# boundless-xyz/boundless

Hardware: AMD Instinct MI355X
Metric: segment-proofs/sec @ 2^20 cycles (higher is better)
Workload: dtype u32 (BabyBear Montgomery)

## Files before the change

boundless_amd/csrc/circuit_dev.hpp:

```cpp
#pragma once
#include <type_traits>

#include "circuit.hpp"
#include "fp.hpp"
#include "poseidon2_arith.hpp"

namespace bx {
inline namespace BX_MAD_FLAVOUR {

constexpr i64 FINAL_MAX = ((i64)(P / 2) - 1) * ((i64)1 << 32);
static_assert(ub(FINAL_MAX) < (i64)P && FINAL_MAX <= SREDC_MAX, "FINAL_MAX");

template <int V>
struct IntC {
    static constexpr int value = V;
};
template <int BEGIN, int END, class F>
BX_HD void static_for(F&& f) {
    if constexpr (BEGIN < END) {
        f(IntC<BEGIN>{});
        static_for<BEGIN + 1, END>(f);
    }
}

template <int TT, int GG>
struct ConsPlan {
    static constexpr int NPOOL = (int)Circuit::POOL;
    static constexpr i64 BC = (i64)(P / 2);
    static constexpr i64 chain_bound() {
        i64 y = BC;
        for (int f = 2; f + 1 < GG; ++f) y = ub(y * BC);
        return y;
    }
    static constexpr i64 TERM = chain_bound() * BC;
    static constexpr int ISZ = (int)(SREDC_MAX / TERM) < 4 ? (int)(SREDC_MAX / TERM) : 4;
    static_assert(ISZ >= 1 && ISZ * TERM <= SREDC_MAX, "cons_sum: inner group beyond sredc's range");

    int nq = 0, no = 0, n2 = 0;
    int first[TT]{}, len[TT]{}, term[TT][ISZ]{};
    int obeg[TT + 1]{}, lbeg[TT + 1]{};
    i64 max_inner = 0, max_outer = 0, max_l2 = 0, max_l3 = 0;

    constexpr ConsPlan() {
        for (int g = 0; g < TT; ++g)
            for (int a = 0; a < NPOOL; ++a) {
                int members[TT]{}, n = 0;
                for (int t = 0; t < TT; ++t)
                    if ((int)Circuit::pool_idx((unsigned)t, 0u) == a) members[n++] = t;
                const int groups = (n + ISZ - 1) / ISZ;
                if (g >= groups) continue;
                const int sz = n / groups + (g < n % groups ? 1 : 0), at = g * (n / groups) + (g < n % groups ? g : n % groups);
                first[nq] = a;
                len[nq] = sz;
                for (int k = 0; k < sz; ++k) term[nq][k] = members[at + k];
                if (sz * TERM > max_inner) max_inner = sz * TERM;
                ++nq;
            }
        i64 rb[TT + 1]{};
        i64 cur = 0;
        for (int q = 0; q < nq; ++q) {
            const i64 add = ub(len[q] * TERM) * BC;
            if (q > 0 && cur + add > SREDC_MAX) {
                rb[no++] = ub(cur);
                obeg[no] = q;
                cur = 0;
            }
            cur += add;
            if (cur > max_outer) max_outer = cur;
        }
        rb[no++] = ub(cur);
        obeg[no] = nq;
        cur = 0;
        for (int o = 0; o < no; ++o) {
            const i64 add = rb[o] * (i64)MONT_ONE;
            if (o > 0 && cur + add > FINAL_MAX) {
                max_l3 += ub(cur) * (i64)MONT_ONE;
                lbeg[++n2] = o;
                cur = 0;
            }
            cur += add;
            if (cur > max_l2) max_l2 = cur;
        }
        max_l3 += ub(cur) * (i64)MONT_ONE;
        lbeg[++n2] = no;
    }
};
template <int TT, int GG>
inline constexpr ConsPlan<TT, GG> cons_plan{};

template <int TT>
struct PairPlan {
    static constexpr int NPOOL = (int)Circuit::POOL, NID = NPOOL * NPOOL;
    static constexpr i64 BC = (i64)(P / 2);
    static constexpr i64 PAIR = ub(BC * BC);
    static constexpr i64 TERM = PAIR * PAIR;
    static constexpr int GRP = (int)(SREDC_MAX / TERM);
    static_assert(GRP == 3 && GRP * TERM <= SREDC_MAX, "cons_sum: pair group beyond sredc's range");
    static constexpr int pair_id(unsigned a, unsigned b) { return a < b ? (int)(a * NPOOL + b) : (int)(b * NPOOL + a); }

    int np = 0, ng = 0, n2 = 0;
    int pa[2 * TT]{}, pb[2 * TT]{};
    int seq[TT]{}, s1[TT]{}, s2[TT]{};
    int pbeg[TT + 1]{};
    int gbeg[TT + 1]{}, lbeg[TT + 1]{};
    int max_live = 0;
    i64 max_group = 0, max_l2 = 0, max_l3 = 0;

    constexpr PairPlan() {
        int sp[TT][3][2]{}, pop[NID]{}, ref[NID]{}, ch[TT]{};
        for (int t = 0; t < TT; ++t) {
            unsigned x[4]{};
            for (unsigned f = 0; f < 4; ++f) x[f] = Circuit::pool_idx((unsigned)t, f);
            for (int s = 0; s < 3; ++s) {
                sp[t][s][0] = pair_id(x[0], x[s + 1]);
                sp[t][s][1] = pair_id(x[s == 0 ? 2 : 1], x[s == 2 ? 2 : 3]);
                ++pop[sp[t][s][0]];
                ++pop[sp[t][s][1]];
            }
        }
        for (int t = 0; t < TT; ++t) {
            for (int s = 1; s < 3; ++s)
                if (pop[sp[t][s][0]] + pop[sp[t][s][1]] > pop[sp[t][ch[t]][0]] + pop[sp[t][ch[t]][1]]) ch[t] = s;
            ++ref[sp[t][ch[t]][0]];
            ++ref[sp[t][ch[t]][1]];
        }
        for (int sweep = 0; sweep < 4; ++sweep)
            for (int t = 0; t < TT; ++t) {
                --ref[sp[t][ch[t]][0]];
                --ref[sp[t][ch[t]][1]];
                int best = 0, best_new = 3, best_ref = 0;
                for (int s = 0; s < 3; ++s) {
                    const int a = sp[t][s][0], b = sp[t][s][1];
                    const int fresh = (ref[a] == 0) + (ref[b] == 0 && b != a), shared = ref[a] + ref[b];
                    if (fresh < best_new || (fresh == best_new && shared > best_ref)) best = s, best_new = fresh, best_ref = shared;
                }
                ch[t] = best;
                ++ref[sp[t][best][0]];
                ++ref[sp[t][best][1]];
            }
        for (int pass = 0; pass < 2; ++pass) {
            int snap[NID]{};
            for (int i = 0; i < NID; ++i) snap[i] = ref[i];
            for (int r = 1; r <= 4; ++r)
                for (int p = 0; p < NID; ++p) {
                    if (snap[p] != r || ref[p] == 0 || ref[p] > 4) continue;
                    int users[4]{}, was[4]{}, nu = 0, moved = 0, delta = 0;
                    for (int t = 0; t < TT; ++t)
                        if (sp[t][ch[t]][0] == p || sp[t][ch[t]][1] == p) users[nu++] = t;
                    for (int u = 0; u < nu; ++u) {
                        was[u] = ch[users[u]];
                        for (int k = 0; k < 2; ++k) delta -= (--ref[sp[users[u]][was[u]][k]] == 0);
                    }
                    for (; moved < nu; ++moved) {
                        const int t = users[moved];
                        int best = -1, best_new = 3, best_ref = 0;
                        for (int s = 0; s < 3; ++s) {
                            const int a = sp[t][s][0], b = sp[t][s][1];
                            if (a == p || b == p) continue;
                            const int fresh = (ref[a] == 0) + (ref[b] == 0 && b != a), shared = ref[a] + ref[b];
                            if (best < 0 || fresh < best_new || (fresh == best_new && shared > best_ref)) best = s, best_new = fresh, best_ref = shared;
                        }
                        if (best < 0) break;
                        ch[t] = best;
                        for (int k = 0; k < 2; ++k) delta += (ref[sp[t][best][k]]++ == 0);
                    }
                    if (moved < nu || delta > 0 || (delta == 0 && pass == 0)) {
                        for (int u = 0; u < moved; ++u)
                            for (int k = 0; k < 2; ++k) --ref[sp[users[u]][ch[users[u]]][k]];
                        for (int u = 0; u < nu; ++u) {
                            ch[users[u]] = was[u];
                            for (int k = 0; k < 2; ++k) ++ref[sp[users[u]][was[u]][k]];
                        }
                    }
                }
        }
        int num[NID]{}, live = 0, glen = 0, gp[2 * GRP]{};
        bool placed[TT]{};
        for (int i = 0; i < NID; ++i) num[i] = -1;
        for (int slot = 0; slot < TT;) {
            int best = -1, best_new = 3, best_last = -1;
            if (glen < GRP)
                for (int t = 0; t < TT; ++t) {
                    if (placed[t]) continue;
                    const int a = sp[t][ch[t]][0], b = sp[t][ch[t]][1];
                    bool clash = false;
                    for (int k = 0; k < 2 * glen; ++k) clash = clash || gp[k] == a || gp[k] == b;
                    if (clash) continue;
                    const int fresh = (num[a] < 0) + (num[b] < 0 && b != a);
                    const int last = a == b ? (ref[a] == 2) : (ref[a] == 1) + (ref[b] == 1);
                    if (fresh < best_new || (fresh == best_new && last > best_last)) best = t, best_new = fresh, best_last = last;
                }
            if (best < 0) {
                gbeg[++ng] = slot;
                glen = 0;
                continue;
            }
            const int a = sp[best][ch[best]][0], b = sp[best][ch[best]][1];
            for (int k = 0; k < 2; ++k) {
                const int id = k ? b : a;
                if (num[id] < 0) {
                    num[id] = np;
                    pa[np] = id / NPOOL;
                    pb[np] = id % NPOOL;
                    ++np;
                    ++live;
                }
            }
            if (live > max_live) max_live = live;
            live -= (--ref[a] == 0);
            live -= (--ref[b] == 0);
            placed[best] = true;
            seq[slot] = best;
            s1[slot] = num[a];
            s2[slot] = num[b];
            gp[2 * glen] = a;
            gp[2 * glen + 1] = b;
            ++glen;
            pbeg[++slot] = np;
        }
        gbeg[++ng] = TT;
        i64 cur = 0;
        for (int g = 0; g < ng; ++g) {
            const i64 sum = (gbeg[g + 1] - gbeg[g]) * TERM, add = ub(sum) * (i64)MONT_ONE;
            if (sum > max_group) max_group = sum;
            if (g > 0 && cur + add > FINAL_MAX) {
                max_l3 += ub(cur) * (i64)MONT_ONE;
                lbeg[++n2] = g;
                cur = 0;
            }
            cur += add;
            if (cur > max_l2) max_l2 = cur;
        }
        max_l3 += ub(cur) * (i64)MONT_ONE;
        lbeg[++n2] = ng;
    }
};
template <int TT>
inline constexpr PairPlan<TT> pair_plan{};

BX_HD i64 smad_r(i32 r, i64 c, int alt = 0) {
#if defined(__HIP_DEVICE_COMPILE__) && defined(BX_PLAIN_MAD)
    (void)alt;
    i32 k = (i32)MONT_ONE;
    asm volatile("" : "+s"(k));
    return (i64)r * (i64)k + c;
#else
    return smad_k(r, MONT_ONE, c, alt);
#endif
}

template <int TT, int GG>
BX_HD uint32_t cons_sum(const i32 (&pool)[Circuit::POOL], uint32_t , uint32_t ) {
    static_assert(TT > 0 && GG > 0, "cons_sum: the run-time form takes a canonical pool");
#pragma unroll
    for (unsigned i = 0; i < Circuit::POOL; ++i) BX_ASSERT_BOUND(pool[i] <= (i32)(P / 2) && pool[i] >= -(i32)(P / 2), "cons_sum: a pool entry that is not centred");
    if constexpr (GG == 4) {
        constexpr int N2 = pair_plan<TT>.n2;
        static_assert(pair_plan<TT>.max_group <= SREDC_MAX, "cons_sum: a group sum beyond sredc's range");
        static_assert(pair_plan<TT>.max_l2 <= FINAL_MAX && pair_plan<TT>.max_l3 <= FINAL_MAX, "cons_sum: term count beyond the three reduction levels");
        i32 pr[pair_plan<TT>.np];
        i64 acc3 = 0;
        i32 result = 0;
        static_for<0, N2>([&](auto lc) {
            constexpr int l = decltype(lc)::value;
            i64 acc2 = 0;
            static_for<pair_plan<TT>.lbeg[l], pair_plan<TT>.lbeg[l + 1]>([&](auto gc) {
                constexpr int g = decltype(gc)::value;
                i64 acc = 0;
                static_for<pair_plan<TT>.gbeg[g], pair_plan<TT>.gbeg[g + 1]>([&](auto sc) {
                    constexpr int s = decltype(sc)::value;
                    static_for<pair_plan<TT>.pbeg[s], pair_plan<TT>.pbeg[s + 1]>([&](auto pc) {
                        constexpr int p = decltype(pc)::value;
                        pr[p] = sredc(smul(pool[pair_plan<TT>.pa[p]], pool[pair_plan<TT>.pb[p]], p), p);
                        BX_ASSERT_BOUND(pr[p] <= PairPlan<TT>::PAIR && pr[p] >= -PairPlan<TT>::PAIR, "cons_sum pair");
                    });
                    acc = smad(pr[pair_plan<TT>.s1[s]], pr[pair_plan<TT>.s2[s]], acc, s);
                });
                acc2 = smad_r(sredc(acc, 3), acc2, g);
            });
            BX_ASSERT_BOUND(acc2 <= FINAL_MAX && acc2 >= -FINAL_MAX, "cons_sum second level");
            const i32 r2 = sredc(acc2, 2);
            if constexpr (N2 == 1) result = r2;
            else acc3 = smad_r(r2, acc3, l);
        });
        if constexpr (N2 > 1) {
            BX_ASSERT_BOUND(acc3 <= FINAL_MAX && acc3 >= -FINAL_MAX, "cons_sum third level");
            result = sredc(acc3, 0);
        }
        return (uint32_t)(result + (result < 0 ? (i32)P : 0));
    } else if constexpr (GG >= 3) {
        constexpr int N2 = cons_plan<TT, GG>.n2;
        static_assert(cons_plan<TT, GG>.max_inner <= SREDC_MAX && cons_plan<TT, GG>.max_outer <= SREDC_MAX, "cons_sum: a group sum beyond sredc's range");
        static_assert(cons_plan<TT, GG>.max_l2 <= FINAL_MAX && cons_plan<TT, GG>.max_l3 <= FINAL_MAX, "cons_sum: term count beyond the three reduction levels");
        i64 acc3 = 0;
        i32 result = 0;
        static_for<0, N2>([&](auto lc) {
            constexpr int l = decltype(lc)::value;
            i64 acc2 = 0;
            static_for<cons_plan<TT, GG>.lbeg[l], cons_plan<TT, GG>.lbeg[l + 1]>([&](auto oc) {
                constexpr int o = decltype(oc)::value;
                i64 outer = 0;
                static_for<cons_plan<TT, GG>.obeg[o], cons_plan<TT, GG>.obeg[o + 1]>([&](auto qc) {
                    constexpr int q = decltype(qc)::value;
                    i64 inner = 0;
                    static_for<0, cons_plan<TT, GG>.len[q]>([&](auto kc) {
                        constexpr int k = decltype(kc)::value;
                        constexpr unsigned t = (unsigned)cons_plan<TT, GG>.term[q][k];
                        i32 y = pool[Circuit::pool_idx(t, 1u)];
#pragma unroll
                        for (int f = 2; f + 1 < GG; ++f) y = sredc(smul(y, pool[Circuit::pool_idx(t, (unsigned)f)], f), f);
                        inner = smad(y, pool[Circuit::pool_idx(t, (unsigned)(GG - 1))], inner, k);
                    });
                    outer = smad(sredc(inner, 3), pool[cons_plan<TT, GG>.first[q]], outer, q);
                });
                acc2 = smad_r(sredc(outer, 1), acc2, o);
            });
            const i32 r2 = sredc(acc2, 2);
            if constexpr (N2 == 1) result = r2;
            else acc3 = smad_r(r2, acc3, l);
        });
        if constexpr (N2 > 1) result = sredc(acc3, 0);
        return (uint32_t)(result + (result < 0 ? (i32)P : 0));
    } else {
        static_assert(TT <= 3 * 8 * 7 && GG >= 1, "cons_sum: term count beyond the three reduction levels");
        constexpr int GRP = 3, NG = (TT + GRP - 1) / GRP;
        i64 acc2 = 0, acc3 = 0;
        i32 result = 0;
#pragma unroll
        for (int g = 0; g < NG; ++g) {
            const int nk = (g + 1) * GRP <= TT ? GRP : TT - g * GRP;
            i64 acc = 0;
#pragma unroll
            for (int k = 0; k < GRP; ++k) {
                if (k < nk) {
                    const i32 x = pool[Circuit::pool_idx((unsigned)(g * GRP + k), 0u)];
                    if constexpr (GG == 1) acc = smad_k(x, MONT_ONE, acc, k);
                    else acc = smad(x, pool[Circuit::pool_idx((unsigned)(g * GRP + k), 1u)], acc, k);
                }
            }
            const i32 r = sredc(acc, 3);
            acc2 = smad_r(r, acc2, g);
            if ((g & 7) == 7 || g == NG - 1) {
                const i32 r2 = sredc(acc2, 1);
                acc2 = 0;
                if constexpr (NG <= 8) result = r2;
                else acc3 = smad_r(r2, acc3, 2);
            }
        }
        if constexpr (NG > 8) result = sredc(acc3, 0);
        return (uint32_t)(result + (result < 0 ? (i32)P : 0));
    }
}

template <int TT, int GG>
BX_HD uint32_t cons_sum(const uint32_t (&pool_u)[Circuit::POOL], uint32_t T, uint32_t G) {
    if constexpr (TT > 0) {
        i32 pool[Circuit::POOL];
#pragma unroll
        for (unsigned i = 0; i < Circuit::POOL; ++i) pool[i] = fp_centre(pool_u[i]);
        return cons_sum<TT, GG>(pool, T, G);
    } else {
        uint32_t sum = 0;
        for (uint32_t t = 0; t < T; ++t) {
            uint32_t prod = pool_u[Circuit::pool_idx(t, 0u)];
            for (uint32_t f = 1; f < G; ++f) prod = fp_mul(prod, pool_u[Circuit::pool_idx(t, f)]);
            sum = fp_add(sum, prod);
        }
        return sum;
    }
}

template <bool CENTRED>
struct DerivedRegs {
    using word = std::conditional_t<CENTRED, i32, uint32_t>;
    BX_HD static word enter(uint32_t v) {
        if constexpr (CENTRED) return fp_centre(v);
        else return v;
    }
    word ring[8], u[3], k[4];
    BX_HD void fill(word (&pool)[Circuit::POOL], word slot1) const {
        pool[0] = u[0]; pool[1] = slot1; pool[2] = u[1]; pool[3] = u[2];
#pragma unroll
        for (int q = 0; q < 8; ++q) pool[4 + q] = ring[q];
#pragma unroll
        for (int q = 0; q < 4; ++q) pool[12 + q] = k[q];
    }
    BX_HD void shift(word d, word next_u, word next_k) {
#pragma unroll
        for (int q = 7; q > 0; --q) ring[q] = ring[q - 1];
        ring[0] = d;
        u[0] = u[1]; u[1] = u[2]; u[2] = next_u;
        k[0] = k[1]; k[1] = k[2]; k[2] = k[3]; k[3] = next_k;
    }
};

}
}
```

Baseline: 30.41.

## Replace multi-level sredc reduction trees in cons_sum with folded i64 accumulator chains

Rewrites all three cons_sum branches (GG==4, GG>=3, GG<=2) to keep one long i64 accumulator chain. Overflow is controlled by a cheap fold_r step, which multiplies the high 32 bits by MONT_ONE and adds the low word, instead of a full sredc at each level. New constexpr planners (FoldPlan, cut_segments) schedule pair products into segments and prove the bounds statically. This removes most intermediate Montgomery reductions in constraint evaluation, but it makes one serial dependence chain where independent group accumulators used to exist, which may lower instruction-level parallelism.

```diff
diff --git a/boundless_amd/csrc/circuit_dev.hpp b/boundless_amd/csrc/circuit_dev.hpp
--- a/boundless_amd/csrc/circuit_dev.hpp
+++ b/boundless_amd/csrc/circuit_dev.hpp
@@ -40,6 +40,8 @@
     int first[TT]{}, len[TT]{}, term[TT][ISZ]{};
     int obeg[TT + 1]{}, lbeg[TT + 1]{};
     i64 max_inner = 0, max_outer = 0, max_l2 = 0, max_l3 = 0;
+    int nf = 0, fbeg[TT + 1]{};
+    i64 max_fchain = 0, max_ftotal = 0;
 
     constexpr ConsPlan() {
         for (int g = 0; g < TT; ++g)
@@ -83,6 +85,27 @@
         }
         max_l3 += ub(cur) * (i64)MONT_ONE;
         lbeg[++n2] = no;
+        const int fewest = cut_segments(nq);
+        if (cut_segments((nq + fewest - 1) / fewest) > fewest) cut_segments(nq);
+    }
+    constexpr int cut_segments(int cap) {
+        i64 cur = 0;
+        nf = 0;
+        max_fchain = 0;
+        for (int q = 0; q < nq; ++q) {
+            const i64 add = ub(len[q] * TERM) * BC;
+            bool again = false;
+            for (int r = fbeg[nf]; r < q; ++r) again = again || first[r] == first[q];
+            if (q > 0 && (again || q - fbeg[nf] >= cap || cur > INT64_MAX - add)) {
+                fbeg[++nf] = q;
+                cur = fold_ub(cur);
+            }
+            cur += add;
+            if (cur > max_fchain) max_fchain = cur;
+        }
+        fbeg[++nf] = nq;
+        max_ftotal = fold_ub(cur);
+        return nf;
     }
 };
 template <int TT, int GG>
@@ -238,6 +261,93 @@
 template <int TT>
 inline constexpr PairPlan<TT> pair_plan{};
 
+template <int TT, int NCH_ = 1>
+struct FoldPlan {
+    static constexpr int SEG = 5, NCH = NCH_;
+    static constexpr i64 TERM = PairPlan<TT>::TERM;
+    static constexpr i64 STEADY = (SEG * TERM + (i64)MONT_ONE + ((i64)1 << 32)) / 15 * 16 + 16;
+    static_assert(NCH >= 1 && STEADY < INT64_MAX && fold_ub(STEADY) + SEG * TERM <= STEADY, "cons_sum: the chain bound is not invariant below 2^63");
+
+    int np = 0, ns = 0;
+    int pa[2 * TT]{}, pb[2 * TT]{};
+    int seq[TT]{}, s1[TT]{}, s2[TT]{};
+    int pbeg[TT + 1]{};
+    int sbeg[TT + 1]{};
+    int max_live = 0;
+    i64 max_chain = 0, max_total = 0;
+
+    constexpr FoldPlan() {
+        const PairPlan<TT>& pp = pair_plan<TT>;
+        int ta[TT]{}, tb[TT]{}, ref[2 * TT]{}, num[2 * TT]{};
+        for (int s = 0; s < TT; ++s) {
+            ta[pp.seq[s]] = pp.s1[s];
+            tb[pp.seq[s]] = pp.s2[s];
+            ++ref[pp.s1[s]];
+            ++ref[pp.s2[s]];
+        }
+        for (int i = 0; i < 2 * TT; ++i) num[i] = -1;
+        int live = 0, glen = 0, gp[2 * SEG]{};
+        bool placed[TT]{};
+        for (int slot = 0; slot < TT;) {
+            int best = -1, best_new = 3, best_last = -1, best_due = 0;
+            const int segs_left = (TT - slot + glen + SEG - 1) / SEG;
+            if (glen < SEG)
+                for (int t = 0; t < TT; ++t) {
+                    if (placed[t]) continue;
+                    const int a = ta[t], b = tb[t];
+                    bool clash = false;
+                    for (int k = 0; k < 2 * glen; ++k) clash = clash || gp[k] == a || gp[k] == b;
+                    if (clash) continue;
+                    const int most = ref[a] > ref[b] ? ref[a] : ref[b], due = most >= segs_left ? most : 0;
+                    const int fresh = (num[a] < 0) + (num[b] < 0 && b != a);
+                    const int last = a == b ? (ref[a] == 2) : (ref[a] == 1) + (ref[b] == 1);
+                    if (due > best_due || (due == best_due && (fresh < best_new || (fresh == best_new && last > best_last))))
+                        best = t, best_new = fresh, best_last = last, best_due = due;
+                }
+            if (best < 0) {
+                sbeg[++ns] = slot;
+                glen = 0;
+                continue;
+            }
+            const int a = ta[best], b = tb[best];
+            for (int k = 0; k < 2; ++k) {
+                const int id = k ? b : a;
+                if (num[id] < 0) {
+                    num[id] = np;
+                    pa[np] = pp.pa[id];
+                    pb[np] = pp.pb[id];
+                    ++np;
+                    ++live;
+                }
+            }
+            if (live > max_live) max_live = live;
+            live -= (--ref[a] == 0);
+            live -= (--ref[b] == 0);
+            placed[best] = true;
+            seq[slot] = best;
+            s1[slot] = num[a];
+            s2[slot] = num[b];
+            gp[2 * glen] = a;
+            gp[2 * glen + 1] = b;
+            ++glen;
+            pbeg[++slot] = np;
+        }
+        sbeg[++ns] = TT;
+        i64 chain[NCH]{};
+        for (int g = 0; g < ns; ++g) {
+            i64& a = chain[g % NCH];
+            a = (g < NCH ? 0 : fold_ub(a)) + (sbeg[g + 1] - sbeg[g]) * TERM;
+            if (a > max_chain) max_chain = a;
+        }
+        for (int c = 0; c < NCH && c < ns; ++c) max_total += fold_ub(chain[c]);
+    }
+};
+template <int TT, int NCH = 1>
+inline constexpr FoldPlan<TT, NCH> fold_plan{};
+constexpr int FOLD_CHAINS = 1;
+template <int TT>
+inline constexpr FoldPlan<TT, FOLD_CHAINS> cons_fold{};
+
 BX_HD i64 smad_r(i32 r, i64 c, int alt = 0) {
 #if defined(__HIP_DEVICE_COMPILE__) && defined(BX_PLAIN_MAD)
     (void)alt;
@@ -249,105 +359,97 @@
 #endif
 }
 
+BX_HD i64 fold_r(i64 a, int alt = 0) {
+    BX_ASSERT_BOUND(a >= -INT64_MAX, "fold_r operand");
+    const i64 r = smad_r((i32)(a >> 32), (i64)(uint32_t)a, alt);
+    BX_ASSERT_BOUND(iabs64(r) <= iabs64(a) / 16 + ((i64)1 << 32) + (i64)MONT_ONE, "fold_r result");
+    return r;
+}
+BX_HD i64 smad_chain(i32 a, i32 b, i64 c, int alt = 0) {
+#if defined(__HIP_DEVICE_COMPILE__) && defined(BX_PLAIN_MAD)
+    (void)alt;
+    i64 r = (i64)a * (i64)b + c;
+    asm("" : "+v"(r));
+    return r;
+#else
+    return smad(a, b, c, alt);
+#endif
+}
+
 template <int TT, int GG>
 BX_HD uint32_t cons_sum(const i32 (&pool)[Circuit::POOL], uint32_t , uint32_t ) {
     static_assert(TT > 0 && GG > 0, "cons_sum: the run-time form takes a canonical pool");
 #pragma unroll
     for (unsigned i = 0; i < Circuit::POOL; ++i) BX_ASSERT_BOUND(pool[i] <= (i32)(P / 2) && pool[i] >= -(i32)(P / 2), "cons_sum: a pool entry that is not centred");
     if constexpr (GG == 4) {
-        constexpr int N2 = pair_plan<TT>.n2;
-        static_assert(pair_plan<TT>.max_group <= SREDC_MAX, "cons_sum: a group sum beyond sredc's range");
-        static_assert(pair_plan<TT>.max_l2 <= FINAL_MAX && pair_plan<TT>.max_l3 <= FINAL_MAX, "cons_sum: term count beyond the three reduction levels");
-        i32 pr[pair_plan<TT>.np];
-        i64 acc3 = 0;
-        i32 result = 0;
-        static_for<0, N2>([&](auto lc) {
-            constexpr int l = decltype(lc)::value;
-            i64 acc2 = 0;
-            static_for<pair_plan<TT>.lbeg[l], pair_plan<TT>.lbeg[l + 1]>([&](auto gc) {
-                constexpr int g = decltype(gc)::value;
-                i64 acc = 0;
-                static_for<pair_plan<TT>.gbeg[g], pair_plan<TT>.gbeg[g + 1]>([&](auto sc) {
-                    constexpr int s = decltype(sc)::value;
-                    static_for<pair_plan<TT>.pbeg[s], pair_plan<TT>.pbeg[s + 1]>([&](auto pc) {
-                        constexpr int p = decltype(pc)::value;
-                        pr[p] = sredc(smul(pool[pair_plan<TT>.pa[p]], pool[pair_plan<TT>.pb[p]], p), p);
-                        BX_ASSERT_BOUND(pr[p] <= PairPlan<TT>::PAIR && pr[p] >= -PairPlan<TT>::PAIR, "cons_sum pair");
-                    });
-                    acc = smad(pr[pair_plan<TT>.s1[s]], pr[pair_plan<TT>.s2[s]], acc, s);
+        using Plan = FoldPlan<TT, FOLD_CHAINS>;
+        constexpr int NCH = Plan::NCH < cons_fold<TT>.ns ? Plan::NCH : cons_fold<TT>.ns;
+        static_assert(cons_fold<TT>.max_chain <= Plan::STEADY, "cons_sum: a chain beyond its steady-state bound");
+        static_assert(cons_fold<TT>.max_total <= FINAL_MAX, "cons_sum: the folded chains beyond the last reduction's range");
+        i32 pr[cons_fold<TT>.np];
+        i64 chain[NCH];
+        static_for<0, cons_fold<TT>.ns>([&](auto gc) {
+            constexpr int g = decltype(gc)::value, c = g % Plan::NCH;
+            static_for<cons_fold<TT>.sbeg[g], cons_fold<TT>.sbeg[g + 1]>([&](auto sc) {
+                constexpr int s = decltype(sc)::value;
+                static_for<cons_fold<TT>.pbeg[s], cons_fold<TT>.pbeg[s + 1]>([&](auto pc) {
+                    constexpr int p = decltype(pc)::value;
+                    pr[p] = sredc(smul(pool[cons_fold<TT>.pa[p]], pool[cons_fold<TT>.pb[p]], p), p);
+                    BX_ASSERT_BOUND(pr[p] <= PairPlan<TT>::PAIR && pr[p] >= -PairPlan<TT>::PAIR, "cons_sum pair");
                 });
-                acc2 = smad_r(sredc(acc, 3), acc2, g);
+                if constexpr (s > cons_fold<TT>.sbeg[g]) chain[c] = smad_chain(pr[cons_fold<TT>.s1[s]], pr[cons_fold<TT>.s2[s]], chain[c], s);
+                else if constexpr (g >= Plan::NCH) chain[c] = smad_chain(pr[cons_fold<TT>.s1[s]], pr[cons_fold<TT>.s2[s]], fold_r(chain[c], g), s);
+                else chain[c] = smul(pr[cons_fold<TT>.s1[s]], pr[cons_fold<TT>.s2[s]], s);
             });
-            BX_ASSERT_BOUND(acc2 <= FINAL_MAX && acc2 >= -FINAL_MAX, "cons_sum second level");
-            const i32 r2 = sredc(acc2, 2);
-            if constexpr (N2 == 1) result = r2;
-            else acc3 = smad_r(r2, acc3, l);
+            BX_ASSERT_BOUND(chain[c] <= cons_fold<TT>.max_chain && chain[c] >= -cons_fold<TT>.max_chain, "cons_sum chain");
         });
-        if constexpr (N2 > 1) {
-            BX_ASSERT_BOUND(acc3 <= FINAL_MAX && acc3 >= -FINAL_MAX, "cons_sum third level");
-            result = sredc(acc3, 0);
-        }
+        i64 total = fold_r(chain[0], 0);
+        static_for<1, NCH>([&](auto cc) { total += fold_r(chain[decltype(cc)::value], decltype(cc)::value); });
+        BX_ASSERT_BOUND(total <= cons_fold<TT>.max_total && total >= -cons_fold<TT>.max_total, "cons_sum folded chains");
+        const i32 result = sredc(total, 0);
         return (uint32_t)(result + (result < 0 ? (i32)P : 0));
     } else if constexpr (GG >= 3) {
-        constexpr int N2 = cons_plan<TT, GG>.n2;
-        static_assert(cons_plan<TT, GG>.max_inner <= SREDC_MAX && cons_plan<TT, GG>.max_outer <= SREDC_MAX, "cons_sum: a group sum beyond sredc's range");
-        static_assert(cons_plan<TT, GG>.max_l2 <= FINAL_MAX && cons_plan<TT, GG>.max_l3 <= FINAL_MAX, "cons_sum: term count beyond the three reduction levels");
-        i64 acc3 = 0;
-        i32 result = 0;
-        static_for<0, N2>([&](auto lc) {
-            constexpr int l = decltype(lc)::value;
-            i64 acc2 = 0;
-            static_for<cons_plan<TT, GG>.lbeg[l], cons_plan<TT, GG>.lbeg[l + 1]>([&](auto oc) {
-                constexpr int o = decltype(oc)::value;
-                i64 outer = 0;
-                static_for<cons_plan<TT, GG>.obeg[o], cons_plan<TT, GG>.obeg[o + 1]>([&](auto qc) {
-                    constexpr int q = decltype(qc)::value;
-                    i64 inner = 0;
-                    static_for<0, cons_plan<TT, GG>.len[q]>([&](auto kc) {
-                        constexpr int k = decltype(kc)::value;
-                        constexpr unsigned t = (unsigned)cons_plan<TT, GG>.term[q][k];
-                        i32 y = pool[Circuit::pool_idx(t, 1u)];
+        static_assert(cons_plan<TT, GG>.max_inner <= SREDC_MAX, "cons_sum: a group sum beyond sredc's range");
+        static_assert(cons_plan<TT, GG>.max_ftotal <= FINAL_MAX, "cons_sum: the folded chain beyond the last reduction's range");
+        i64 chain = 0;
+        static_for<0, cons_plan<TT, GG>.nf>([&](auto fc) {
+            constexpr int f = decltype(fc)::value;
+            static_for<cons_plan<TT, GG>.fbeg[f], cons_plan<TT, GG>.fbeg[f + 1]>([&](auto qc) {
+                constexpr int q = decltype(qc)::value;
+                i64 inner = 0;
+                static_for<0, cons_plan<TT, GG>.len[q]>([&](auto kc) {
+                    constexpr int k = decltype(kc)::value;
+                    constexpr unsigned t = (unsigned)cons_plan<TT, GG>.term[q][k];
+                    i32 y = pool[Circuit::pool_idx(t, 1u)];
 #pragma unroll
-                        for (int f = 2; f + 1 < GG; ++f) y = sredc(smul(y, pool[Circuit::pool_idx(t, (unsigned)f)], f), f);
-                        inner = smad(y, pool[Circuit::pool_idx(t, (unsigned)(GG - 1))], inner, k);
-                    });
-                    outer = smad(sredc(inner, 3), pool[cons_plan<TT, GG>.first[q]], outer, q);
+                    for (int g = 2; g + 1 < GG; ++g) y = sredc(smul(y, pool[Circuit::pool_idx(t, (unsigned)g)], g), g);
+                    inner = smad_chain(y, pool[Circuit::pool_idx(t, (unsigned)(GG - 1))], inner, k);
                 });
-                acc2 = smad_r(sredc(outer, 1), acc2, o);
+                const i32 s = sredc(inner, 3);
+                if constexpr (q > cons_plan<TT, GG>.fbeg[f]) chain = smad_chain(s, pool[cons_plan<TT, GG>.first[q]], chain, q);
+                else if constexpr (f > 0) chain = smad_chain(s, pool[cons_plan<TT, GG>.first[q]], fold_r(chain, f), q);
+                else chain = smul(s, pool[cons_plan<TT, GG>.first[q]], q);
             });
-            const i32 r2 = sredc(acc2, 2);
-            if constexpr (N2 == 1) result = r2;
-            else acc3 = smad_r(r2, acc3, l);
+            BX_ASSERT_BOUND(iabs64(chain) <= (cons_plan<TT, GG>.max_fchain), "cons_sum chain");
         });
-        if constexpr (N2 > 1) result = sredc(acc3, 0);
+        const i32 result = sredc(fold_r(chain, 0), 0);
         return (uint32_t)(result + (result < 0 ? (i32)P : 0));
     } else {
-        static_assert(TT <= 3 * 8 * 7 && GG >= 1, "cons_sum: term count beyond the three reduction levels");
-        constexpr int GRP = 3, NG = (TT + GRP - 1) / GRP;
-        i64 acc2 = 0, acc3 = 0;
-        i32 result = 0;
-#pragma unroll
-        for (int g = 0; g < NG; ++g) {
-            const int nk = (g + 1) * GRP <= TT ? GRP : TT - g * GRP;
-            i64 acc = 0;
-#pragma unroll
-            for (int k = 0; k < GRP; ++k) {
-                if (k < nk) {
-                    const i32 x = pool[Circuit::pool_idx((unsigned)(g * GRP + k), 0u)];
-                    if constexpr (GG == 1) acc = smad_k(x, MONT_ONE, acc, k);
-                    else acc = smad(x, pool[Circuit::pool_idx((unsigned)(g * GRP + k), 1u)], acc, k);
-                }
-            }
-            const i32 r = sredc(acc, 3);
-            acc2 = smad_r(r, acc2, g);
-            if ((g & 7) == 7 || g == NG - 1) {
-                const i32 r2 = sredc(acc2, 1);
-                acc2 = 0;
-                if constexpr (NG <= 8) result = r2;
-                else acc3 = smad_r(r2, acc3, 2);
-            }
-        }
-        if constexpr (NG > 8) result = sredc(acc3, 0);
+        constexpr int SEG2 = 8;
+        constexpr i64 TERM = (i64)(P / 2) * (GG == 1 ? (i64)MONT_ONE : (i64)(P / 2));
+        constexpr i64 STEADY = (SEG2 * TERM + (i64)MONT_ONE + ((i64)1 << 32)) / 15 * 16 + 16;
+        static_assert(GG >= 1 && STEADY < INT64_MAX && fold_ub(STEADY) + SEG2 * TERM <= STEADY && fold_ub(STEADY) <= FINAL_MAX, "cons_sum: the chain bound is not invariant below 2^63");
+        i64 chain = 0;
+        static_for<0, TT>([&](auto tc) {
+            constexpr unsigned t = (unsigned)decltype(tc)::value;
+            const i32 x = pool[Circuit::pool_idx(t, 0u)];
+            if constexpr (t > 0 && t % SEG2 == 0) chain = fold_r(chain, (int)t);
+            if constexpr (GG == 1) chain = smad_r(x, chain, (int)t);
+            else if constexpr (t == 0) chain = smul(x, pool[Circuit::pool_idx(t, 1u)], 0);
+            else chain = smad_chain(x, pool[Circuit::pool_idx(t, 1u)], chain, (int)t);
+            BX_ASSERT_BOUND(chain <= STEADY && chain >= -STEADY, "cons_sum chain");
+        });
+        const i32 result = sredc(fold_r(chain, 0), 0);
         return (uint32_t)(result + (result < 0 ? (i32)P : 0));
     }
 }
```

After: 31.30 (median of 6 runs). +2.9%, better.
